# DreamWaterFound/self_commit_ORB-SLAM2

Measured on AMD Instinct MI355X. Metric: frames/s ORB extract+match (1000 feat, 640x480), higher is better.
Workload: dtype u8; 1 GPU; batch of 256 synthetic 640x480 frames per GPU (8 distinct resident batches per step, one launch set per batch), ORB extract (1000 feat, 8 levels, FAST 20/7) + brute-force Hamming SearchByBoW of consecutive frames; batch_per_gpu=256, streams=3, width=640, height=480, nfeatures=1000, parallelism=frames sharded, 1 rank(s), no data-path collective

## Files before the change

### self_commit_orb-slam2_amd/csrc/orbx_match.hip

```cpp
#include <math.h>
#include <string.h>

#include <atomic>
#include <chrono>

#include <type_traits>
#include <vector>

#include "orbx_match_internal.h"

using namespace orbx_match;

namespace {

__global__ __launch_bounds__(256) void k_bow_order(FeatDev A, const int32_t *__restrict__ pairsA, int32_t *__restrict__ order, int stride)
{
    const int p = blockIdx.y, fa = pairsA[p];
    const int nA = min(A.counts[fa], A.cap);
    const int i = blockIdx.x * 256 + threadIdx.x;
    if (i >= nA) return;
    int32_t *ord = order + (size_t)p * stride;
    if (!A.groups) { ord[i] = i; return; }
    const int32_t *g = A.groups + (size_t)fa * A.cap;
    const int gi = g[i];
    int rank = 0;
    for (int k = 0; k < nA; k++) { int gk = g[k]; rank += (gk < gi) || (gk == gi && k < i); }
    ord[rank] = i;
}

#define TOPK_NROW 1
#define TOPK_ROWS (256 * TOPK_NROW)
#define TOPK_TILE 1024

__device__ __forceinline__ uint32_t bcnt_acc(uint32_t x, uint32_t acc)
{
    uint32_t r;
    asm("v_bcnt_u32_b32 %0, %1, %2" : "=v"(r) : "v"(x), "v"(acc));
    return r;
}

struct TriDev {
    const float *f12;
    const float *epipole;
    const uint8_t *stereoA, *stereoB;
    float epiTh[ORBX_MAX_LEVELS];
    double chiTh[ORBX_MAX_LEVELS];
};

__device__ __forceinline__ bool tri_geom_ok(const TriDev &T, int p, const orbx_keypoint &k1, bool st1, const orbx_keypoint &k2, bool st2)
{
    if (!st1 && !st2) {
        const float distex = T.epipole[2 * p] - k2.x, distey = T.epipole[2 * p + 1] - k2.y;
        if (distex * distex + distey * distey < T.epiTh[k2.octave]) return false;
    }
    const float *F = T.f12 + 9 * p;
    const float a = k1.x * F[0] + k1.y * F[3] + F[6];
    const float b = k1.x * F[1] + k1.y * F[4] + F[7];
    const float c = k1.x * F[2] + k1.y * F[5] + F[8];
    const float num = a * k2.x + b * k2.y + c;
    const float den = a * a + b * b;
    if (den == 0) return false;
    const float dsqr = num * num / den;
    return (double)dsqr < T.chiTh[k2.octave];
}

__device__ __forceinline__ uint32_t med3_u32(uint32_t a, uint32_t b, uint32_t c)
{
    uint32_t r;
    asm("v_med3_u32 %0, %1, %2, %3" : "=v"(r) : "v"(a), "v"(b), "v"(c));
    return r;
}

__device__ __forceinline__ void topk_insert(uint32_t (&kk)[TOPK], uint32_t key)
{
#pragma unroll
    for (int q = TOPK - 1; q > 0; q--) kk[q] = med3_u32(kk[q - 1], kk[q], key);
    kk[0] = min(kk[0], key);
}

template <bool FILTER, bool TRI, int NROW>
__global__ __launch_bounds__(256) void k_bow_topk(FeatDev A, FeatDev B, const int32_t *__restrict__ pairsA, const int32_t *__restrict__ pairsB, int mode,
                                                  uint32_t dcut, uint32_t *__restrict__ topk, int stride, TriDev T)
{
    __shared__ uint4 sB[TOPK_TILE * 2];
    __shared__ int32_t sG[TOPK_TILE];
    const int p = blockIdx.y, fa = pairsA[p], fb = pairsB[p];
    const int nA = min(A.counts[fa], A.cap), nB = min(B.counts[fb], B.cap);
    const int capB = B.cap;
    const int row0 = blockIdx.x * (256 * NROW);
    if (row0 >= nA) return;
    const int tid = threadIdx.x;
    int ir[NROW];
    bool live[NROW], act[NROW];
    uint32_t a[NROW][8], kk[NROW][TOPK], th[NROW];
    int gA[NROW];
    const uint32_t sentinel = dcut << 16;
#pragma unroll
    for (int r = 0; r < NROW; r++) {
        ir[r] = row0 + 256 * r + tid;
        live[r] = ir[r] < nA;
        const size_t ia = (size_t)fa * A.cap + (live[r] ? ir[r] : nA - 1);
        const uint32_t *da = (const uint32_t *)(A.desc + ia * 32);
#pragma unroll
        for (int w = 0; w < 8; w++) a[r][w] = da[w];
        gA[r] = (FILTER && A.groups) ? A.groups[ia] : 0;
        act[r] = live[r] && !(FILTER && gA[r] < 0);
#pragma unroll
        for (int q = 0; q < TOPK; q++) kk[r][q] = act[r] ? sentinel : 0u;
        th[r] = kk[r][TOPK - 1] >> 16;
    }
    const uint4 *gD = (const uint4 *)(B.desc + (size_t)fb * capB * 32);
    for (int t0base = 0; t0base < nB; t0base += TOPK_TILE) {
        const int nt = min(TOPK_TILE, nB - t0base), ntPad = (nt + 3) & ~3;
        __syncthreads();
        for (int t = tid; t < 2 * ntPad; t += 256) sB[t] = t < 2 * nt ? gD[2 * (size_t)t0base + t] : make_uint4(0u, 0u, 0u, 0u);
        if (FILTER)
            for (int j = tid; j < ntPad; j += 256) {
                int gq = (int)0x80000000;
                if (j < nt) {
                    gq = B.groups ? B.groups[(size_t)fb * capB + t0base + j] : 0;
                    if (gq < 0) gq = (int)0x80000000;
                    if (mode >= 1 && B.valid && !B.valid[(size_t)fb * capB + t0base + j]) gq = (int)0x80000000;
                }
                sG[j] = gq;
            }
        __syncthreads();
        auto group = [&](const int j0, auto tailTag) {
            constexpr bool TAIL = decltype(tailTag)::value;
            uint32_t dd[NROW][4];
#pragma unroll
            for (int u = 0; u < 4; u++) {
                const uint4 lo = sB[2 * (j0 + u)], hi = sB[2 * (j0 + u) + 1];
                const uint32_t bw[8] = {lo.x, lo.y, lo.z, lo.w, hi.x, hi.y, hi.z, hi.w};
                uint32_t d[NROW];
#pragma unroll
                for (int r = 0; r < NROW; r++) d[r] = bcnt_acc(a[r][0] ^ bw[0], 0u);
#pragma unroll
                for (int w = 1; w < 8; w++)
#pragma unroll
                    for (int r = 0; r < NROW; r++) d[r] = bcnt_acc(a[r][w] ^ bw[w], d[r]);
                if (FILTER) {
                    const int gq = sG[j0 + u];
#pragma unroll
                    for (int r = 0; r < NROW; r++) d[r] = gq == gA[r] ? d[r] : 0xffffu;
                } else if (TAIL && j0 + u >= nt) {
#pragma unroll
                    for (int r = 0; r < NROW; r++) d[r] = 0xffffu;
                }
#pragma unroll
                for (int r = 0; r < NROW; r++) dd[r][u] = d[r];
            }
            auto reaches = [](uint32_t d, uint32_t t) { return TRI ? d <= t : d < t; };
            bool any4 = false;
#pragma unroll
            for (int r = 0; r < NROW; r++) any4 = any4 || reaches(min(min(dd[r][0], min(dd[r][1], dd[r][2])), dd[r][3]), th[r]);
            if (__any(any4)) {
#pragma unroll
                for (int u = 0; u < 4; u++) {
                    bool anyU = false;
#pragma unroll
                    for (int r = 0; r < NROW; r++) anyU = anyU || reaches(dd[r][u], th[r]);
                    if (__any(anyU)) {
                        const uint32_t j = TRI ? 0xffffu - (uint32_t)(t0base + j0 + u) : (uint32_t)(t0base + j0 + u);
                        uint32_t ins[NROW];
#pragma unroll
                        for (int r = 0; r < NROW; r++) ins[r] = (dd[r][u] << 16) | j;
                        if (TRI) {
                            const int jb = t0base + j0 + u;
                            const orbx_keypoint k2 = B.kp[(size_t)fb * capB + jb];
                            const bool st2 = T.stereoB && T.stereoB[(size_t)fb * capB + jb];
#pragma unroll
                            for (int r = 0; r < NROW; r++) {
                                bool pass = false;
                                if (ins[r] < kk[r][TOPK - 1]) {
                                    const size_t ia = (size_t)fa * A.cap + ir[r];
                                    pass = tri_geom_ok(T, p, A.kp[ia], T.stereoA && T.stereoA[ia], k2, st2);
                                }
                                ins[r] = pass ? ins[r] : 0xffffffffu;
                            }
                        }
#pragma unroll
                        for (int r = 0; r < NROW; r++)
                            if (__any(ins[r] < kk[r][TOPK - 1])) { topk_insert(kk[r], ins[r]); th[r] = kk[r][TOPK - 1] >> 16; }
                    }
                }
            }
        };
        int j0 = 0;
        for (; j0 + 4 <= nt; j0 += 4) group(j0, std::false_type());
        if (j0 < ntPad) group(j0, std::true_type());
    }
#pragma unroll
    for (int r = 0; r < NROW; r++)
        if (live[r]) {
            uint32_t *out = topk + ((size_t)p * stride + ir[r]) * TOPK;
#pragma unroll
            for (int k = 0; k < TOPK; k++) out[k] = (!act[r] || kk[r][k] >= sentinel) ? KEY_EMPTY : kk[r][k];
        }
}

typedef int mfma_v4i __attribute__((ext_vector_type(4)));
typedef int mfma_v16i __attribute__((ext_vector_type(16)));

__device__ __forceinline__ uint32_t nib01(uint32_t n) { return __umul24(n, 0x00204081u) & 0x01010101u; }

__global__ __launch_bounds__(256, 3) void k_bow_topk_mfma(FeatDev A, FeatDev B, const int32_t *__restrict__ pairsA, const int32_t *__restrict__ pairsB, uint32_t dcut,
                                                       uint32_t *__restrict__ topk, int stride, int dbg)
{
    __shared__ uint32_t sLut[16 * 64];
    const int p = blockIdx.y, fa = pairsA[p], fb = pairsB[p];
    const int nA = min(A.counts[fa], A.cap), nB = min(B.counts[fb], B.cap);
    const int capB = B.cap;
    const int row0 = blockIdx.x * 256;
    if (row0 >= nA) return;
    const int tid = threadIdx.x, lane = tid & 63, wv = tid >> 6, g = lane >> 5, c = lane & 31;
    for (int e = tid; e < 16 * 64; e += 256) sLut[e] = nib01((uint32_t)e >> 6);
    __syncthreads();
    if (row0 + 64 * wv >= nA) return;
    const uint32_t sentinel = dcut << 16;
    const char *lut = (const char *)sLut;
    const uint32_t lane4 = (uint32_t)lane << 2;
    mfma_v4i a[2][8];
    uint32_t kk[2][TOPK];
    int iA[2], nAc[2], T[2];
    bool live[2];
#pragma unroll
    for (int s = 0; s < 2; s++) {
        iA[s] = row0 + 64 * wv + 32 * s + c;
        live[s] = iA[s] < nA;
        const uint4 *da = (const uint4 *)(A.desc + ((size_t)fa * A.cap + (live[s] ? iA[s] : nA - 1)) * 32);
        const uint4 lo = da[0], hi = da[1];
        nAc[s] = __popc(lo.x) + __popc(lo.y) + __popc(lo.z) + __popc(lo.w) + __popc(hi.x) + __popc(hi.y) + __popc(hi.z) + __popc(hi.w);
        const uint4 mine = g ? hi : lo;
        const uint32_t w[4] = {mine.x, mine.y, mine.z, mine.w};
#pragma unroll
        for (int t = 0; t < 8; t++) {
            const uint32_t two = (w[t >> 1] >> (16 * (t & 1))) & 0xffffu;
#pragma unroll
            for (int q = 0; q < 4; q++) a[s][t][q] = (int)__builtin_amdgcn_perm(0u, 0x0000ff01u, nib01((two >> (4 * q)) & 15u));
        }
#pragma unroll
        for (int q = 0; q < TOPK; q++) kk[s][q] = live[s] ? sentinel : 0u;
        T[s] = (int)(kk[s][TOPK - 1] >> 16) - nAc[s];
    }
    const uint4 *gD = (const uint4 *)(B.desc + (size_t)fb * capB * 32);
    const int ntiles = (nB + 31) >> 5;
    auto load_raw = [&](int tile) { const int j = tile * 32 + c; return j < nB ? gD[(size_t)j * 2 + g] : make_uint4(0u, 0u, 0u, 0u); };
    uint4 raw = load_raw(0);
    auto one_tile = [&](const int tile, auto lastTag) {
        constexpr bool LAST = decltype(lastTag)::value;
// ... 802 lines not shown
    int ndev = 0;
    if (hipGetDeviceCount(&ndev) != hipSuccess || ndev <= 0) { orbx_set_error("no HIP device available: liborbx has no CPU fallback"); return ORBX_ERR_NODEVICE; }
    if (device < 0 || device >= ndev) { orbx_set_error("device %d out of range", device); return ORBX_ERR_ARG; }
    ORBX_HIP_CHECK(hipSetDevice(device));
    orbx_matcher *m = new orbx_matcher();
    m->device = device; m->maxFeatures = max_features; m->maxPairs = max_pairs;
    if (hipStreamCreateWithFlags(&m->stream, hipStreamNonBlocking) != hipSuccess) { delete m; orbx_set_error("hipStreamCreate failed"); return ORBX_ERR_HIP; }
    (void)hipEventCreateWithFlags(&m->evDep, hipEventDisableTiming);
    (void)hipEventCreateWithFlags(&m->evDep2, hipEventDisableTiming);
    (void)hipEventCreateWithFlags(&m->evPyr[0], hipEventDisableTiming);
    (void)hipEventCreateWithFlags(&m->evPyr[1], hipEventDisableTiming);
    (void)hipEventCreateWithFlags(&m->evDone[0], hipEventDisableTiming);
    (void)hipEventCreateWithFlags(&m->evDone[1], hipEventDisableTiming);
    for (int r = 0; r < MATCH_PROF_RING; r++) { (void)hipEventCreate(&m->ev0[r]); (void)hipEventCreate(&m->ev1[r]); (void)hipEventCreate(&m->evMid[r]); }
    const size_t S = (size_t)max_features, P = (size_t)max_pairs;
    int rc;
    if ((rc = m->pairsA.ensure(P)) || (rc = m->pairsB.ensure(P)) || (rc = m->order.ensure(P * S)) || (rc = m->matches.ensure(P * S)) ||
        (rc = m->dists.ensure(P * S)) || (rc = m->nmatches.ensure(P)) || (rc = m->topk.ensure(P * S * TOPK)) || (rc = m->scales.ensure(128)) ||
        (rc = m->uright.ensure(P * S)) || (rc = m->depth.ensure(P * S)) || (rc = m->sad.ensure(P * S))) {
        orbx_matcher_destroy(m);
        return rc;
    }
    *out = m;
    return ORBX_OK;
}

extern "C" void orbx_matcher_destroy(orbx_matcher *m)
{
    if (!m) return;
    (void)hipSetDevice(m->device);
    if (m->stream) (void)hipStreamSynchronize(m->stream);
    m->pairsA.release(); m->pairsB.release(); m->order.release(); m->matches.release(); m->dists.release(); m->nmatches.release();
    m->hostStage.release(); m->projDec.release(); m->projQueue.release(); m->box.release(); m->arena.release();
    m->topk.release(); m->scales.release(); m->uright.release(); m->depth.release(); m->sad.release(); m->stRowStart.release(); m->stRowList.release();
    m->topk64.release(); m->pkp.release(); m->producerStatus.release();
    for (int q = 0; q < 2; q++) { m->pf[q].release(); m->pb[q].release(); m->pi32[q].release(); }
    if (m->evDep2) (void)hipEventDestroy(m->evDep2);
    m->sfZero.release(); m->sfScalesDev.release();
    if (m->sfHost) (void)hipHostFree(m->sfHost);
    for (int i = 0; i < 2; i++) if (m->evPyr[i]) (void)hipEventDestroy(m->evPyr[i]);
    for (int s = 0; s < 2; s++) { m->hk[s].release(); m->hd[s].release(); m->hv[s].release(); m->hc[s].release(); m->hg[s].release(); m->hs[s].release(); }
    m->triGeom.release(); m->frProj.release(); m->frLevel.release(); m->frInView.release();
    if (m->evDep) (void)hipEventDestroy(m->evDep);
    for (int i = 0; i < 2; i++) if (m->evDone[i]) (void)hipEventDestroy(m->evDone[i]);
    for (int r = 0; r < MATCH_PROF_RING; r++) { if (m->ev0[r]) (void)hipEventDestroy(m->ev0[r]); if (m->ev1[r]) (void)hipEventDestroy(m->ev1[r]); if (m->evMid[r]) (void)hipEventDestroy(m->evMid[r]); }
    if (m->stream) (void)hipStreamDestroy(m->stream);
    delete m;
}

__global__ void k_status_or(int *dst, const int *src, int first) { if (first) *dst = *src; else if (*src) atomicOr(dst, *src); }

namespace orbx_match {

int inherit_status(orbx_matcher *m, orbx_extractor *after, bool first)
{
    if (!after) return ORBX_OK;
    const int *w = orbx_extractor_status_word_internal(after);
    if (!w) return ORBX_OK;
    if (!m->producerStatus.p) {
        int rc = m->producerStatus.ensure(1);
        if (rc != ORBX_OK) return rc;
        ORBX_HIP_CHECK(hipMemsetAsync(m->producerStatus.p, 0, sizeof(int), m->stream));
    }
    hipLaunchKernelGGL(k_status_or, dim3(1), dim3(1), 0, m->stream, m->producerStatus.p, w, first ? 1 : 0);
    return ORBX_OK;
}

int check_producer_status(orbx_matcher *m)
{
    if (!m->producerStatus.p) return ORBX_OK;
    int v = 0;
    ORBX_HIP_CHECK(hipMemcpy(&v, m->producerStatus.p, sizeof(int), hipMemcpyDeviceToHost));
    if (!v) return ORBX_OK;
    ORBX_HIP_CHECK(hipMemset(m->producerStatus.p, 0, sizeof(int)));
    orbx_set_error("the extractor batch these results were computed from overflowed a device capacity (bits 0x%x: 1 = >%d FAST candidates in a level, "
                   "2 = quadtree node list, 4 = level keypoints): results are not the reference's", v, 32768);
    return ORBX_ERR_CAPACITY;
}

int prep_pairs(orbx_matcher *m, const orbx_feature_set *a, const orbx_feature_set *b, const int32_t *pa, const int32_t *pb, int npairs,
                      orbx_extractor *after)
{
    if (!m || !a || !b || !pa || !pb) { orbx_set_error("NULL argument"); return ORBX_ERR_ARG; }
    if (npairs < 1 || npairs > m->maxPairs) { orbx_set_error("npairs %d outside 1..%d", npairs, m->maxPairs); return ORBX_ERR_CAPACITY; }
    if (a->capacity > m->maxFeatures || b->capacity > m->maxFeatures || a->capacity < 1 || b->capacity < 1) {
        orbx_set_error("feature capacity %d/%d exceeds the matcher's max_features %d", a->capacity, b->capacity, m->maxFeatures);
        return ORBX_ERR_CAPACITY;
    }
    if (!a->keypoints || !a->descriptors || !a->counts || !b->keypoints || !b->descriptors || !b->counts) { orbx_set_error("NULL feature arrays"); return ORBX_ERR_ARG; }
    for (int p = 0; p < npairs; p++)
        if (pa[p] < 0 || pa[p] >= a->nframes || pb[p] < 0 || pb[p] >= b->nframes) { orbx_set_error("pair %d references a frame out of range", p); return ORBX_ERR_ARG; }
    ORBX_HIP_CHECK(hipSetDevice(m->device));
    if (after) {
        ORBX_HIP_CHECK(hipEventRecord(m->evDep, orbx_extractor_stream_internal(after)));
        ORBX_HIP_CHECK(hipStreamWaitEvent(m->stream, m->evDep, 0));
        int rcs = inherit_status(m, after, true);
        if (rcs != ORBX_OK) return rcs;
    } else if (m->producerStatus.p)
        ORBX_HIP_CHECK(hipMemsetAsync(m->producerStatus.p, 0, sizeof(int), m->stream));
    ORBX_HIP_CHECK(hipMemcpyAsync(m->pairsA.p, pa, (size_t)npairs * sizeof(int32_t), hipMemcpyHostToDevice, m->stream));
    ORBX_HIP_CHECK(hipMemcpyAsync(m->pairsB.p, pb, (size_t)npairs * sizeof(int32_t), hipMemcpyHostToDevice, m->stream));
    return ORBX_OK;
}

int chain_back(orbx_matcher *m, orbx_extractor *after)
{
    if (!after) return ORBX_OK;
    hipEvent_t ev = m->evDone[m->doneSlot];
    m->doneSlot ^= 1;
    ORBX_HIP_CHECK(hipEventRecord(ev, m->stream));
    orbx_extractor_set_consumer_event_internal(after, ev);
    return ORBX_OK;
}

FeatDev to_dev(const orbx_feature_set *s)
{
    FeatDev f;
    f.kp = s->keypoints; f.desc = s->descriptors; f.counts = s->counts; f.groups = s->groups; f.valid = s->valid; f.cap = s->capacity;
    return f;
}

}

extern "C" int orbx_search_by_bow_device(orbx_matcher *m, const orbx_feature_set *a, const orbx_feature_set *b, const int32_t *pairs_a,
                                         const int32_t *pairs_b, int npairs, const orbx_bow_params *params, orbx_extractor *after)
{
    if (!params || (params->mode != 0 && params->mode != 1)) { orbx_set_error("bad bow params"); return ORBX_ERR_ARG; }
    int rc = prep_pairs(m, a, b, pairs_a, pairs_b, npairs, after);
    if (rc != ORBX_OK) return rc;
    const int stride = m->maxFeatures;
    FeatDev A = to_dev(a), B = to_dev(b);
    const int slot = m->profCount % MATCH_PROF_RING;
    ORBX_HIP_CHECK(hipEventRecord(m->ev0[slot], m->stream));
    uint32_t dcut = TH_LOW + 1;
    while (dcut < 257 && !(params->nn_ratio * (float)dcut > (float)TH_LOW)) dcut++;
    const bool filter = b->groups != nullptr || (params->mode == 1 && b->valid != nullptr);
    const dim3 gridTopk((unsigned)((a->capacity + TOPK_ROWS - 1) / TOPK_ROWS), (unsigned)npairs);
    if (filter)
        hipLaunchKernelGGL((k_bow_topk<true, false, TOPK_NROW>), gridTopk, dim3(256), 0, m->stream, A, B, m->pairsA.p, m->pairsB.p, params->mode, dcut, m->topk.p, stride, TriDev());
    else {
        const char *em = getenv("ORBX_MATCH_MFMA");
        const bool mfma = em && em[0] == '1';
        static const int dbg = getenv("ORBX_MFMA_DEBUG") ? atoi(getenv("ORBX_MFMA_DEBUG")) : 0;
        if (mfma) hipLaunchKernelGGL(k_bow_topk_mfma, dim3((unsigned)((a->capacity + 255) / 256), (unsigned)npairs), dim3(256), 0, m->stream, A, B, m->pairsA.p, m->pairsB.p, dcut, m->topk.p, stride, dbg);
        else hipLaunchKernelGGL((k_bow_topk<false, false, TOPK_NROW>), gridTopk, dim3(256), 0, m->stream, A, B, m->pairsA.p, m->pairsB.p, params->mode, dcut, m->topk.p, stride, TriDev());
    }
    MLAUNCH_CHECK();
    ORBX_HIP_CHECK(hipEventRecord(m->evMid[slot], m->stream));
    m->midValid[slot] = true;
    hipLaunchKernelGGL(k_bow_order, dim3((unsigned)((a->capacity + 255) / 256), (unsigned)npairs), dim3(256), 0, m->stream, A, m->pairsA.p, m->order.p, stride);
    MLAUNCH_CHECK();
    const size_t ldsGreedy = (size_t)b->capacity * 4 + (size_t)a->capacity * 4 + (size_t)((a->capacity + 7) & ~7) * 2 * 2;
    if (ldsGreedy > 160 * 1024) { orbx_set_error("feature capacity %d too large for the LDS tile", a->capacity); return ORBX_ERR_CAPACITY; }
    if (ldsGreedy > 48 * 1024) ORBX_HIP_CHECK(hipFuncSetAttribute((const void *)k_bow_greedy, hipFuncAttributeMaxDynamicSharedMemorySize, (int)ldsGreedy));
    hipLaunchKernelGGL(k_bow_greedy, dim3((unsigned)npairs), dim3(GREEDY_THREADS), ldsGreedy, m->stream, A, B, m->pairsA.p, m->pairsB.p, params->mode, params->nn_ratio,
                       params->check_orientation, m->topk.p, m->order.p, m->matches.p, m->dists.p, m->nmatches.p, stride, TriDev(), (int32_t *)nullptr, (unsigned long long *)nullptr, 0ull);
    MLAUNCH_CHECK();
    ORBX_HIP_CHECK(hipEventRecord(m->ev1[slot], m->stream));
    m->profCount++;
    m->lastPairs = npairs; m->lastStride = stride;
    return chain_back(m, after);
}

extern "C" int orbx_stereo_match_device(orbx_matcher *m, const orbx_feature_set *left, const orbx_feature_set *right, const int32_t *pairs_l,
                                        const int32_t *pairs_r, int npairs, const float *scale_factors, int nlevels, float max_disparity,
                                        orbx_extractor *after)
{
    if (!scale_factors || nlevels < 1 || nlevels > 64) { orbx_set_error("bad scale factor table"); return ORBX_ERR_ARG; }
    int rc = prep_pairs(m, left, right, pairs_l, pairs_r, npairs, after);
    if (rc != ORBX_OK) return rc;
    const int stride = m->maxFeatures;
    ORBX_HIP_CHECK(hipMemcpyAsync(m->scales.p, scale_factors, (size_t)nlevels * sizeof(float), hipMemcpyHostToDevice, m->stream));
    ORBX_HIP_CHECK(hipMemsetAsync(m->nmatches.p, 0, (size_t)npairs * sizeof(int32_t), m->stream));
    const int slot = m->profCount % MATCH_PROF_RING;
    ORBX_HIP_CHECK(hipEventRecord(m->ev0[slot], m->stream));
    m->midValid[slot] = false;
    hipLaunchKernelGGL(k_stereo, dim3((unsigned)((left->capacity + 3) / 4), (unsigned)npairs), dim3(256), 0, m->stream, to_dev(left), to_dev(right), m->pairsA.p,
                       m->pairsB.p, m->scales.p, max_disparity, m->matches.p, m->dists.p, m->nmatches.p, stride);
    MLAUNCH_CHECK();
    ORBX_HIP_CHECK(hipEventRecord(m->ev1[slot], m->stream));
    m->profCount++;
    m->lastPairs = npairs; m->lastStride = stride;
    return chain_back(m, after);
}

extern "C" int orbx_compute_stereo_matches_device(orbx_matcher *m, orbx_extractor *left, orbx_extractor *right, const int32_t *frames_l,
                                                  const int32_t *frames_r, int npairs, float mbf, float mb)
{
    if (!m || !left || !right || !frames_l || !frames_r) { orbx_set_error("NULL argument"); return ORBX_ERR_ARG; }
    OrbxLastBatchView vl, vr;
    int rc;
    if ((rc = orbx_extractor_last_batch_view_internal(left, &vl)) != ORBX_OK || (rc = orbx_extractor_last_batch_view_internal(right, &vr)) != ORBX_OK) return rc;
    if (vl.nlevels != vr.nlevels || vl.geom->W != vr.geom->W || vl.geom->H != vr.geom->H) {
        orbx_set_error("left and right extractors differ in geometry (%dx%d/%d vs %dx%d/%d)", vl.geom->W, vl.geom->H, vl.nlevels, vr.geom->W, vr.geom->H, vr.nlevels);
        return ORBX_ERR_ARG;
    }
    if (vl.nlevels > 64) { orbx_set_error("too many levels"); return ORBX_ERR_ARG; }
    orbx_feature_set fl = {vl.kp, vl.desc, vl.counts, nullptr, nullptr, vl.cap, vl.batch};
    orbx_feature_set fr = {vr.kp, vr.desc, vr.counts, nullptr, nullptr, vr.cap, vr.batch};
    rc = prep_pairs(m, &fl, &fr, frames_l, frames_r, npairs, left);
    if (rc != ORBX_OK) return rc;
    if (right != left) {
        ORBX_HIP_CHECK(hipEventRecord(m->evDep2, orbx_extractor_stream_internal(right)));
        ORBX_HIP_CHECK(hipStreamWaitEvent(m->stream, m->evDep2, 0));
// ... 337 lines not shown
    if ((rc = bx.wait(m->stream)) != ORBX_OK) return rc;
    const int32_t *res = bx.outHost<int32_t>(0);
    if (nOut > 0) memcpy(matches, res, (size_t)nOut * 4);
    *nmatches = res[nOut];
    return ORBX_OK;
}

extern "C" int orbx_search_by_bow(orbx_matcher *m, const orbx_feature_set *a_host, const orbx_feature_set *b_host, const orbx_bow_params *params,
                                  int32_t *matches, int32_t *nmatches)
{
    if (!m || !matches || !nmatches) { orbx_set_error("NULL argument"); return ORBX_ERR_ARG; }
    if (!params || (params->mode != 0 && params->mode != 1)) { orbx_set_error("bad bow params"); return ORBX_ERR_ARG; }
    ORBX_HIP_CHECK(hipSetDevice(m->device));
    static const bool split = !(getenv("ORBX_BOW_SINGLE_SPLIT") && getenv("ORBX_BOW_SINGLE_SPLIT")[0] == '0');
    if (split && a_host && b_host && a_host->keypoints && a_host->descriptors && a_host->counts && b_host->keypoints && b_host->descriptors && b_host->counts &&
        a_host->counts[0] > 0 && b_host->counts[0] > 0 && a_host->counts[0] <= m->maxFeatures && b_host->counts[0] <= std::min(m->maxFeatures, 4000))
        return search_by_bow_single(m, a_host, b_host, params, matches, nmatches);
    orbx_feature_set da, db;
    int rc;
    if ((rc = stage_host(m, 0, a_host, &da)) != ORBX_OK || (rc = stage_host(m, 1, b_host, &db)) != ORBX_OK) return rc;
    const int32_t zero = 0;
    if ((rc = orbx_search_by_bow_device(m, &da, &db, &zero, &zero, 1, params, nullptr)) != ORBX_OK) return rc;
    ORBX_HIP_CHECK(hipStreamSynchronize(m->stream));
    const int nOut = params->mode == 0 ? b_host->counts[0] : a_host->counts[0];
    if (nOut > 0) ORBX_HIP_CHECK(hipMemcpy(matches, m->matches.p, (size_t)nOut * 4, hipMemcpyDeviceToHost));
    ORBX_HIP_CHECK(hipMemcpy(nmatches, m->nmatches.p, 4, hipMemcpyDeviceToHost));
    return ORBX_OK;
}

extern "C" int orbx_search_for_triangulation_device(orbx_matcher *m, const orbx_feature_set *a, const orbx_feature_set *b, const int32_t *pairs_a,
                                                    const int32_t *pairs_b, int npairs, const orbx_triangulation_params *params, orbx_extractor *after)
{
    if (!params || !params->f12 || !params->epipole || !params->scale_factors || !params->level_sigma2) { orbx_set_error("bad triangulation params"); return ORBX_ERR_ARG; }
    if (params->nlevels < 1 || params->nlevels > ORBX_MAX_LEVELS) { orbx_set_error("nlevels %d outside 1..%d", params->nlevels, ORBX_MAX_LEVELS); return ORBX_ERR_ARG; }
    int rc = prep_pairs(m, a, b, pairs_a, pairs_b, npairs, after);
    if (rc != ORBX_OK) return rc;
    if ((rc = m->triGeom.ensure((size_t)11 * m->maxPairs)) != ORBX_OK) return rc;
    ORBX_HIP_CHECK(hipMemcpyAsync(m->triGeom.p, params->f12, (size_t)9 * npairs * sizeof(float), hipMemcpyHostToDevice, m->stream));
    ORBX_HIP_CHECK(hipMemcpyAsync(m->triGeom.p + (size_t)9 * m->maxPairs, params->epipole, (size_t)2 * npairs * sizeof(float), hipMemcpyHostToDevice, m->stream));
    TriDev T = TriDev();
    T.f12 = m->triGeom.p; T.epipole = m->triGeom.p + (size_t)9 * m->maxPairs;
    T.stereoA = params->stereo_a; T.stereoB = params->stereo_b;
    for (int l = 0; l < params->nlevels; l++) {
        T.epiTh[l] = 100 * params->scale_factors[l];
        T.chiTh[l] = 3.84 * params->level_sigma2[l];
    }
    const int stride = m->maxFeatures;
    FeatDev A = to_dev(a), B = to_dev(b);
    const int slot = m->profCount % MATCH_PROF_RING;
    ORBX_HIP_CHECK(hipEventRecord(m->ev0[slot], m->stream));
    hipLaunchKernelGGL(k_bow_order, dim3((unsigned)((a->capacity + 255) / 256), (unsigned)npairs), dim3(256), 0, m->stream, A, m->pairsA.p, m->order.p, stride);
    MLAUNCH_CHECK();
    const dim3 gridTopk((unsigned)((a->capacity + TOPK_ROWS - 1) / TOPK_ROWS), (unsigned)npairs);
    hipLaunchKernelGGL((k_bow_topk<true, true, TOPK_NROW>), gridTopk, dim3(256), 0, m->stream, A, B, m->pairsA.p, m->pairsB.p, 2, (uint32_t)(TH_LOW + 1), m->topk.p, stride, T);
    MLAUNCH_CHECK();
    m->midValid[slot] = false;
    const size_t ldsGreedy = (size_t)b->capacity * 4 + (size_t)a->capacity * 4 + (size_t)((a->capacity + 7) & ~7) * 2 * 2;
    if (ldsGreedy > 160 * 1024) { orbx_set_error("feature capacity %d too large for the LDS tile", a->capacity); return ORBX_ERR_CAPACITY; }
    if (ldsGreedy > 48 * 1024) ORBX_HIP_CHECK(hipFuncSetAttribute((const void *)k_bow_greedy, hipFuncAttributeMaxDynamicSharedMemorySize, (int)ldsGreedy));
    hipLaunchKernelGGL(k_bow_greedy, dim3((unsigned)npairs), dim3(GREEDY_THREADS), ldsGreedy, m->stream, A, B, m->pairsA.p, m->pairsB.p, 2, 0.0f, params->check_orientation,
                       m->topk.p, m->order.p, m->matches.p, m->dists.p, m->nmatches.p, stride, T, (int32_t *)nullptr, (unsigned long long *)nullptr, 0ull);
    MLAUNCH_CHECK();
    ORBX_HIP_CHECK(hipEventRecord(m->ev1[slot], m->stream));
    m->profCount++;
    m->lastPairs = npairs; m->lastStride = stride;
    return chain_back(m, after);
}

extern "C" int orbx_search_for_triangulation(orbx_matcher *m, const orbx_feature_set *a_host, const orbx_feature_set *b_host,
                                             const orbx_triangulation_params *params_host, int32_t *matches12, int32_t *nmatches)
{
    if (!m || !params_host || !matches12 || !nmatches) { orbx_set_error("NULL argument"); return ORBX_ERR_ARG; }
    ORBX_HIP_CHECK(hipSetDevice(m->device));
    orbx_feature_set da, db;
    int rc;
    if ((rc = stage_host(m, 0, a_host, &da)) != ORBX_OK || (rc = stage_host(m, 1, b_host, &db)) != ORBX_OK) return rc;
    orbx_triangulation_params P = *params_host;
    const uint8_t *hostFlags[2] = {params_host->stereo_a, params_host->stereo_b};
    const int cnt[2] = {a_host->counts[0], b_host->counts[0]};
    const uint8_t *devFlags[2] = {nullptr, nullptr};
    for (int sd = 0; sd < 2; sd++) {
        if (!hostFlags[sd]) continue;
        if ((rc = m->hs[sd].ensure((size_t)m->maxFeatures)) != ORBX_OK) return rc;
        if (cnt[sd] > 0) ORBX_HIP_CHECK(hipMemcpyAsync(m->hs[sd].p, hostFlags[sd], (size_t)cnt[sd], hipMemcpyHostToDevice, m->stream));
        devFlags[sd] = m->hs[sd].p;
    }
    P.stereo_a = devFlags[0]; P.stereo_b = devFlags[1];
    const int32_t zero = 0;
    if ((rc = orbx_search_for_triangulation_device(m, &da, &db, &zero, &zero, 1, &P, nullptr)) != ORBX_OK) return rc;
    ORBX_HIP_CHECK(hipStreamSynchronize(m->stream));
    if (cnt[0] > 0) ORBX_HIP_CHECK(hipMemcpy(matches12, m->matches.p, (size_t)cnt[0] * 4, hipMemcpyDeviceToHost));
    ORBX_HIP_CHECK(hipMemcpy(nmatches, m->nmatches.p, 4, hipMemcpyDeviceToHost));
    return ORBX_OK;
}

extern "C" int orbx_stereo_match(orbx_matcher *m, const orbx_feature_set *left_host, const orbx_feature_set *right_host, const float *scale_factors,
                                 int nlevels, float max_disparity, int32_t *best_dist, int32_t *best_idx)
{
    if (!m || !best_dist || !best_idx) { orbx_set_error("NULL argument"); return ORBX_ERR_ARG; }
    ORBX_HIP_CHECK(hipSetDevice(m->device));
    orbx_feature_set dl, dr;
    int rc;
    if ((rc = stage_host(m, 0, left_host, &dl)) != ORBX_OK || (rc = stage_host(m, 1, right_host, &dr)) != ORBX_OK) return rc;
    const int32_t zero = 0;
    if ((rc = orbx_stereo_match_device(m, &dl, &dr, &zero, &zero, 1, scale_factors, nlevels, max_disparity, nullptr)) != ORBX_OK) return rc;
    ORBX_HIP_CHECK(hipStreamSynchronize(m->stream));
    const int nL = left_host->counts[0];
// ... 7 lines not shown
```

### self_commit_orb-slam2_amd/csrc/orbx_match_internal.h

```cpp
#ifndef ORBX_MATCH_INTERNAL_H
#define ORBX_MATCH_INTERNAL_H

#include "orbx_internal.h"

#define TH_HIGH 100
#define TH_LOW 50
#define HISTO_LENGTH 30
#define KEY_EMPTY 0xffffffffu
#define TOPK 8
#define MATCH_PROF_RING 64

#define KEY64_EMPTY 0xffffffffffffffffull
#define GRID_COLS 64
#define GRID_ROWS 48

struct FeatDev {
    const orbx_keypoint *kp;
    const uint8_t *desc;
    const int32_t *counts;
    const int32_t *groups;
    const uint8_t *valid;
    int cap;
};

// ... 42 lines not shown
struct orbx_matcher {
    int device = 0, maxFeatures = 0, maxPairs = 0;
    hipStream_t stream = nullptr;
    hipEvent_t evDep = nullptr, evDone[2] = {nullptr, nullptr};
    int doneSlot = 0;
    hipEvent_t ev0[MATCH_PROF_RING] = {}, ev1[MATCH_PROF_RING] = {};
    hipEvent_t evMid[MATCH_PROF_RING] = {};
    bool midValid[MATCH_PROF_RING] = {};
    float lastDistanceMs = 0.f, lastReplayMs = 0.f;
    int profCount = 0;
    OrbxDevBuf<int32_t> pairsA, pairsB, order, matches, dists, nmatches;
    OrbxDevBuf<uint32_t> topk;
    OrbxDevBuf<float> scales, uright, depth, pf[2];
    OrbxDevBuf<unsigned long long> topk64;
    OrbxDevBuf<uint8_t> pb[2];
    OrbxDevBuf<int32_t> pi32[2];
    OrbxDevBuf<orbx_keypoint> pkp;
    OrbxDevBuf<uint32_t> projDec, projQueue;
    OrbxHostStage hostStage;
    OrbxCallBox box;
    OrbxDevBuf<uint8_t> arena;
    OrbxDevBuf<int32_t> sad;
    OrbxDevBuf<int32_t> stRowStart, stRowList;
    hipEvent_t evDep2 = nullptr, evPyr[2] = {nullptr, nullptr};
    int lastStereoPairs = 0;
    float sfScales[128] = {};
    int sfLevels = 0;
    OrbxDevBuf<int32_t> sfZero;
    OrbxDevBuf<float> sfScalesDev;
    float *sfHost = nullptr, *sfHostDev = nullptr;
    size_t sfHostFloats = 0;
    int sfSeq = 0, sfFlagSeq = 0;
    int sfPending = 0;
    OrbxDevBuf<orbx_keypoint> hk[2];
    OrbxDevBuf<uint8_t> hd[2], hv[2];
    OrbxDevBuf<int32_t> hc[2], hg[2];
    OrbxDevBuf<uint8_t> hs[2];
    OrbxDevBuf<float> triGeom;
    OrbxDevBuf<float> frProj;
    OrbxDevBuf<int32_t> frLevel;
    OrbxDevBuf<uint8_t> frInView;
    size_t frCount = 0;
    int lastPairs = 0, lastStride = 0;
    OrbxDevBuf<int> producerStatus;
};

#define MLAUNCH_CHECK()                                                                                              \
    do {                                                                                                             \
        hipError_t e_ = hipGetLastError();                                                                           \
        if (e_ != hipSuccess) { orbx_set_error("kernel launch failed: %s (%s:%d)", hipGetErrorString(e_), __FILE__, __LINE__); return ORBX_ERR_HIP; } \
    } while (0)

namespace orbx_match {
int prep_pairs(orbx_matcher *m, const orbx_feature_set *a, const orbx_feature_set *b, const int32_t *pa, const int32_t *pb, int npairs, orbx_extractor *after);
int chain_back(orbx_matcher *m, orbx_extractor *after);
int inherit_status(orbx_matcher *m, orbx_extractor *after, bool first = true);
int check_producer_status(orbx_matcher *m);
FeatDev to_dev(const orbx_feature_set *s);
int stage_host(orbx_matcher *m, int side, const orbx_feature_set *h, orbx_feature_set *d);
}

#endif
```

Before: 307,500 frames/s.

## Stream B descriptors through scalar loads and fold order/status kernels into top-k

Adds a default unfiltered top-k path that reads frame-B descriptors through wave-uniform scalar (constant address space) loads, double-buffered across groups of four, in place of staging 1024-descriptor tiles in LDS behind barriers. The top-k kernel now also writes the identity order and copies the producer status word, so the separate k_bow_order and k_status_or launches are skipped when there are no groups. This cuts LDS traffic, block barriers and two small launches per batch, but relies on scalar cache bandwidth and manual waitcnt handling. The LDS path remains available through an environment flag.

```diff
diff --git a/self_commit_orb-slam2_amd/csrc/orbx_match.hip b/self_commit_orb-slam2_amd/csrc/orbx_match.hip
--- a/self_commit_orb-slam2_amd/csrc/orbx_match.hip
+++ b/self_commit_orb-slam2_amd/csrc/orbx_match.hip
@@ -29,6 +29,7 @@
 }
 
 #define TOPK_NROW 1
+#define TOPK_SNROW 1
 #define TOPK_ROWS (256 * TOPK_NROW)
 #define TOPK_TILE 1024
 
@@ -78,18 +79,95 @@
     kk[0] = min(kk[0], key);
 }
 
-template <bool FILTER, bool TRI, int NROW>
+typedef uint32_t topk_u32x8 __attribute__((ext_vector_type(8), aligned(4)));
+__device__ __forceinline__ void topk_sload4(uint32_t (&s)[32], const uint8_t *base, int j, int last)
+{
+#pragma unroll
+    for (int u = 0; u < 4; u++) {
+        const int idx = __builtin_amdgcn_readfirstlane(min(j + u, last));
+        const topk_u32x8 v = *(const volatile __attribute__((address_space(4))) topk_u32x8 *)(uintptr_t)(base + (size_t)idx * 32);
+#pragma unroll
+        for (int w = 0; w < 8; w++) s[8 * u + w] = v[w];
+    }
+}
+
+template <bool FILTER, bool TRI, int NROW, bool TAIL, class FetchB, class NodeB>
+__device__ __forceinline__ void topk_group(const uint32_t (&a)[NROW][8], const int (&gA)[NROW], const int (&ir)[NROW], uint32_t (&kk)[NROW][TOPK], uint32_t (&th)[NROW],
+                                           const int jb, const int nLeft, FetchB fetchB, NodeB nodeB, const FeatDev &A, const FeatDev &B, const int fa, const int fb,
+                                           const int p, const TriDev &T)
+{
+    uint32_t dd[NROW][4];
+#pragma unroll
+    for (int u = 0; u < 4; u++) {
+        uint32_t bw[8];
+        fetchB(u, bw);
+        uint32_t d[NROW];
+#pragma unroll
+        for (int r = 0; r < NROW; r++) d[r] = bcnt_acc(a[r][0] ^ bw[0], 0u);
+#pragma unroll
+        for (int w = 1; w < 8; w++)
+#pragma unroll
+            for (int r = 0; r < NROW; r++) d[r] = bcnt_acc(a[r][w] ^ bw[w], d[r]);
+        if (FILTER) {
+            const int gq = nodeB(u);
+#pragma unroll
+            for (int r = 0; r < NROW; r++) d[r] = gq == gA[r] ? d[r] : 0xffffu;
+        } else if (TAIL && u >= nLeft) {
+#pragma unroll
+            for (int r = 0; r < NROW; r++) d[r] = 0xffffu;
+        }
+#pragma unroll
+        for (int r = 0; r < NROW; r++) dd[r][u] = d[r];
+    }
+    auto reaches = [](uint32_t d, uint32_t t) { return TRI ? d <= t : d < t; };
+    bool any4 = false;
+#pragma unroll
+    for (int r = 0; r < NROW; r++) any4 = any4 || reaches(min(min(dd[r][0], min(dd[r][1], dd[r][2])), dd[r][3]), th[r]);
+    if (__any(any4)) {
+#pragma unroll
+        for (int u = 0; u < 4; u++) {
+            bool anyU = false;
+#pragma unroll
+            for (int r = 0; r < NROW; r++) anyU = anyU || reaches(dd[r][u], th[r]);
+            if (__any(anyU)) {
+                const uint32_t j = TRI ? 0xffffu - (uint32_t)(jb + u) : (uint32_t)(jb + u);
+                uint32_t ins[NROW];
+#pragma unroll
+                for (int r = 0; r < NROW; r++) ins[r] = (dd[r][u] << 16) | j;
+                if (TRI) {
+                    const orbx_keypoint k2 = B.kp[(size_t)fb * B.cap + jb + u];
+                    const bool st2 = T.stereoB && T.stereoB[(size_t)fb * B.cap + jb + u];
+#pragma unroll
+                    for (int r = 0; r < NROW; r++) {
+                        bool pass = false;
+                        if (ins[r] < kk[r][TOPK - 1]) {
+                            const size_t ia = (size_t)fa * A.cap + ir[r];
+                            pass = tri_geom_ok(T, p, A.kp[ia], T.stereoA && T.stereoA[ia], k2, st2);
+                        }
+                        ins[r] = pass ? ins[r] : 0xffffffffu;
+                    }
+                }
+#pragma unroll
+                for (int r = 0; r < NROW; r++)
+                    if (__any(ins[r] < kk[r][TOPK - 1])) { topk_insert(kk[r], ins[r]); th[r] = kk[r][TOPK - 1] >> 16; }
+            }
+        }
+    }
+}
+
+template <bool FILTER, bool TRI, int NROW, bool SCALAR>
 __global__ __launch_bounds__(256) void k_bow_topk(FeatDev A, FeatDev B, const int32_t *__restrict__ pairsA, const int32_t *__restrict__ pairsB, int mode,
-                                                  uint32_t dcut, uint32_t *__restrict__ topk, int stride, TriDev T)
-{
-    __shared__ uint4 sB[TOPK_TILE * 2];
-    __shared__ int32_t sG[TOPK_TILE];
+                                                  uint32_t dcut, uint32_t *__restrict__ topk, int stride, TriDev T, int32_t *__restrict__ order,
+                                                  int *__restrict__ statDst, const int *__restrict__ statSrc)
+{
+    static_assert(!SCALAR || (!FILTER && !TRI), "the scalar body is the unfiltered search");
+    const int tid = threadIdx.x;
+    if (statSrc && blockIdx.x == 0 && blockIdx.y == 0 && tid == 0) *statDst = *statSrc;
     const int p = blockIdx.y, fa = pairsA[p], fb = pairsB[p];
     const int nA = min(A.counts[fa], A.cap), nB = min(B.counts[fb], B.cap);
     const int capB = B.cap;
     const int row0 = blockIdx.x * (256 * NROW);
     if (row0 >= nA) return;
-    const int tid = threadIdx.x;
     int ir[NROW];
     bool live[NROW], act[NROW];
     uint32_t a[NROW][8], kk[NROW][TOPK], th[NROW];
@@ -109,86 +187,61 @@
         for (int q = 0; q < TOPK; q++) kk[r][q] = act[r] ? sentinel : 0u;
         th[r] = kk[r][TOPK - 1] >> 16;
     }
-    const uint4 *gD = (const uint4 *)(B.desc + (size_t)fb * capB * 32);
-    for (int t0base = 0; t0base < nB; t0base += TOPK_TILE) {
-        const int nt = min(TOPK_TILE, nB - t0base), ntPad = (nt + 3) & ~3;
-        __syncthreads();
-        for (int t = tid; t < 2 * ntPad; t += 256) sB[t] = t < 2 * nt ? gD[2 * (size_t)t0base + t] : make_uint4(0u, 0u, 0u, 0u);
-        if (FILTER)
-            for (int j = tid; j < ntPad; j += 256) {
-                int gq = (int)0x80000000;
-                if (j < nt) {
-                    gq = B.groups ? B.groups[(size_t)fb * capB + t0base + j] : 0;
-                    if (gq < 0) gq = (int)0x80000000;
-                    if (mode >= 1 && B.valid && !B.valid[(size_t)fb * capB + t0base + j]) gq = (int)0x80000000;
+    if constexpr (SCALAR) {
+        const uint8_t *gB = B.desc + (size_t)fb * capB * 32;
+        const int last = nB - 1;
+        uint32_t s0[32], s1[32];
+        auto none = [](int) { return 0; };
+        auto step = [&](uint32_t (&cur)[32], uint32_t (&nxt)[32], const int j0, auto tailTag) {
+            __builtin_amdgcn_s_waitcnt(0xc07f);
+            topk_sload4(nxt, gB, j0 + 4, last);
+            topk_group<false, false, NROW, decltype(tailTag)::value>(a, gA, ir, kk, th, j0, nB - j0, [&](int u, uint32_t (&bw)[8]) {
+#pragma unroll
+                for (int w = 0; w < 8; w++) bw[w] = cur[8 * u + w];
+            }, none, A, B, fa, fb, p, T);
+        };
+        if (nB > 0) {
+            topk_sload4(s0, gB, 0, last);
+            int j0 = 0;
+            for (; j0 + 8 <= nB; j0 += 8) {
+                step(s0, s1, j0, std::false_type());
+                step(s1, s0, j0 + 4, std::false_type());
+            }
+            if (j0 + 4 <= nB) {
+                step(s0, s1, j0, std::false_type());
+                if (j0 + 4 < nB) step(s1, s0, j0 + 4, std::true_type());
+            } else if (j0 < nB)
+                step(s0, s1, j0, std::true_type());
+        }
+    } else {
+        __shared__ uint4 sB[TOPK_TILE * 2];
+        __shared__ int32_t sG[TOPK_TILE];
+        const uint4 *gD = (const uint4 *)(B.desc + (size_t)fb * capB * 32);
+        for (int t0base = 0; t0base < nB; t0base += TOPK_TILE) {
+            const int nt = min(TOPK_TILE, nB - t0base), ntPad = (nt + 3) & ~3;
+            __syncthreads();
+            for (int t = tid; t < 2 * ntPad; t += 256) sB[t] = t < 2 * nt ? gD[2 * (size_t)t0base + t] : make_uint4(0u, 0u, 0u, 0u);
+            if (FILTER)
+                for (int j = tid; j < ntPad; j += 256) {
+                    int gq = (int)0x80000000;
+                    if (j < nt) {
+                        gq = B.groups ? B.groups[(size_t)fb * capB + t0base + j] : 0;
+                        if (gq < 0) gq = (int)0x80000000;
+                        if (mode >= 1 && B.valid && !B.valid[(size_t)fb * capB + t0base + j]) gq = (int)0x80000000;
+                    }
+                    sG[j] = gq;
                 }
-                sG[j] = gq;
-            }
-        __syncthreads();
-        auto group = [&](const int j0, auto tailTag) {
-            constexpr bool TAIL = decltype(tailTag)::value;
-            uint32_t dd[NROW][4];
-#pragma unroll
-            for (int u = 0; u < 4; u++) {
-                const uint4 lo = sB[2 * (j0 + u)], hi = sB[2 * (j0 + u) + 1];
-                const uint32_t bw[8] = {lo.x, lo.y, lo.z, lo.w, hi.x, hi.y, hi.z, hi.w};
-                uint32_t d[NROW];
-#pragma unroll
-                for (int r = 0; r < NROW; r++) d[r] = bcnt_acc(a[r][0] ^ bw[0], 0u);
-#pragma unroll
-                for (int w = 1; w < 8; w++)
-#pragma unroll
-                    for (int r = 0; r < NROW; r++) d[r] = bcnt_acc(a[r][w] ^ bw[w], d[r]);
-                if (FILTER) {
-                    const int gq = sG[j0 + u];
-#pragma unroll
-                    for (int r = 0; r < NROW; r++) d[r] = gq == gA[r] ? d[r] : 0xffffu;
-                } else if (TAIL && j0 + u >= nt) {
-#pragma unroll
-                    for (int r = 0; r < NROW; r++) d[r] = 0xffffu;
-                }
-#pragma unroll
-                for (int r = 0; r < NROW; r++) dd[r][u] = d[r];
-            }
-            auto reaches = [](uint32_t d, uint32_t t) { return TRI ? d <= t : d < t; };
-            bool any4 = false;
-#pragma unroll
-            for (int r = 0; r < NROW; r++) any4 = any4 || reaches(min(min(dd[r][0], min(dd[r][1], dd[r][2])), dd[r][3]), th[r]);
-            if (__any(any4)) {
-#pragma unroll
-                for (int u = 0; u < 4; u++) {
-                    bool anyU = false;
-#pragma unroll
-                    for (int r = 0; r < NROW; r++) anyU = anyU || reaches(dd[r][u], th[r]);
-                    if (__any(anyU)) {
-                        const uint32_t j = TRI ? 0xffffu - (uint32_t)(t0base + j0 + u) : (uint32_t)(t0base + j0 + u);
-                        uint32_t ins[NROW];
-#pragma unroll
-                        for (int r = 0; r < NROW; r++) ins[r] = (dd[r][u] << 16) | j;
-                        if (TRI) {
-                            const int jb = t0base + j0 + u;
-                            const orbx_keypoint k2 = B.kp[(size_t)fb * capB + jb];
-                            const bool st2 = T.stereoB && T.stereoB[(size_t)fb * capB + jb];
-#pragma unroll
-                            for (int r = 0; r < NROW; r++) {
-                                bool pass = false;
-                                if (ins[r] < kk[r][TOPK - 1]) {
-                                    const size_t ia = (size_t)fa * A.cap + ir[r];
-                                    pass = tri_geom_ok(T, p, A.kp[ia], T.stereoA && T.stereoA[ia], k2, st2);
-                                }
-                                ins[r] = pass ? ins[r] : 0xffffffffu;
-                            }
-                        }
-#pragma unroll
-                        for (int r = 0; r < NROW; r++)
-                            if (__any(ins[r] < kk[r][TOPK - 1])) { topk_insert(kk[r], ins[r]); th[r] = kk[r][TOPK - 1] >> 16; }
-                    }
-                }
-            }
-        };
-        int j0 = 0;
-        for (; j0 + 4 <= nt; j0 += 4) group(j0, std::false_type());
-        if (j0 < ntPad) group(j0, std::true_type());
+            __syncthreads();
+            auto group = [&](const int j0, auto tailTag) {
+                topk_group<FILTER, TRI, NROW, decltype(tailTag)::value>(a, gA, ir, kk, th, t0base + j0, nt - j0, [&](int u, uint32_t (&bw)[8]) {
+                    const uint4 lo = sB[2 * (j0 + u)], hi = sB[2 * (j0 + u) + 1];
+                    bw[0] = lo.x; bw[1] = lo.y; bw[2] = lo.z; bw[3] = lo.w; bw[4] = hi.x; bw[5] = hi.y; bw[6] = hi.z; bw[7] = hi.w;
+                }, [&](int u) { return sG[j0 + u]; }, A, B, fa, fb, p, T);
+            };
+            int j0 = 0;
+            for (; j0 + 4 <= nt; j0 += 4) group(j0, std::false_type());
+            if (j0 < ntPad) group(j0, std::true_type());
+        }
     }
 #pragma unroll
     for (int r = 0; r < NROW; r++)
@@ -196,6 +249,7 @@
             uint32_t *out = topk + ((size_t)p * stride + ir[r]) * TOPK;
 #pragma unroll
             for (int k = 0; k < TOPK; k++) out[k] = (!act[r] || kk[r][k] >= sentinel) ? KEY_EMPTY : kk[r][k];
+            if (order && !A.groups) order[(size_t)p * stride + ir[r]] = ir[r];
         }
 }
 
@@ -1104,7 +1158,7 @@
 
 namespace orbx_match {
 
-int inherit_status(orbx_matcher *m, orbx_extractor *after, bool first)
+int inherit_status(orbx_matcher *m, orbx_extractor *after, bool first, const int **deferred)
 {
     if (!after) return ORBX_OK;
     const int *w = orbx_extractor_status_word_internal(after);
@@ -1114,6 +1168,7 @@
         if (rc != ORBX_OK) return rc;
         ORBX_HIP_CHECK(hipMemsetAsync(m->producerStatus.p, 0, sizeof(int), m->stream));
     }
+    if (deferred && first) { *deferred = w; return ORBX_OK; }
     hipLaunchKernelGGL(k_status_or, dim3(1), dim3(1), 0, m->stream, m->producerStatus.p, w, first ? 1 : 0);
     return ORBX_OK;
 }
@@ -1131,8 +1186,9 @@
 }
 
 int prep_pairs(orbx_matcher *m, const orbx_feature_set *a, const orbx_feature_set *b, const int32_t *pa, const int32_t *pb, int npairs,
-                      orbx_extractor *after)
-{
+                      orbx_extractor *after, const int **deferredStatus)
+{
+    if (deferredStatus) *deferredStatus = nullptr;
     if (!m || !a || !b || !pa || !pb) { orbx_set_error("NULL argument"); return ORBX_ERR_ARG; }
     if (npairs < 1 || npairs > m->maxPairs) { orbx_set_error("npairs %d outside 1..%d", npairs, m->maxPairs); return ORBX_ERR_CAPACITY; }
     if (a->capacity > m->maxFeatures || b->capacity > m->maxFeatures || a->capacity < 1 || b->capacity < 1) {
@@ -1146,7 +1202,7 @@
     if (after) {
         ORBX_HIP_CHECK(hipEventRecord(m->evDep, orbx_extractor_stream_internal(after)));
         ORBX_HIP_CHECK(hipStreamWaitEvent(m->stream, m->evDep, 0));
-        int rcs = inherit_status(m, after, true);
+        int rcs = inherit_status(m, after, true, deferredStatus);
         if (rcs != ORBX_OK) return rcs;
     } else if (m->producerStatus.p)
         ORBX_HIP_CHECK(hipMemsetAsync(m->producerStatus.p, 0, sizeof(int), m->stream));
@@ -1178,7 +1234,11 @@
                                          const int32_t *pairs_b, int npairs, const orbx_bow_params *params, orbx_extractor *after)
 {
     if (!params || (params->mode != 0 && params->mode != 1)) { orbx_set_error("bad bow params"); return ORBX_ERR_ARG; }
-    int rc = prep_pairs(m, a, b, pairs_a, pairs_b, npairs, after);
+    const bool filter = a && b && (b->groups != nullptr || (params->mode == 1 && b->valid != nullptr));
+    const char *em = getenv("ORBX_MATCH_MFMA"), *el = getenv("ORBX_TOPK_LDS");
+    const bool mfma = !filter && em && em[0] == '1', lds = el && el[0] == '1';
+    const int *statSrc = nullptr;
+    int rc = prep_pairs(m, a, b, pairs_a, pairs_b, npairs, after, mfma ? nullptr : &statSrc);
     if (rc != ORBX_OK) return rc;
     const int stride = m->maxFeatures;
     FeatDev A = to_dev(a), B = to_dev(b);
@@ -1186,22 +1246,27 @@
     ORBX_HIP_CHECK(hipEventRecord(m->ev0[slot], m->stream));
     uint32_t dcut = TH_LOW + 1;
     while (dcut < 257 && !(params->nn_ratio * (float)dcut > (float)TH_LOW)) dcut++;
-    const bool filter = b->groups != nullptr || (params->mode == 1 && b->valid != nullptr);
     const dim3 gridTopk((unsigned)((a->capacity + TOPK_ROWS - 1) / TOPK_ROWS), (unsigned)npairs);
+    int *const statDst = m->producerStatus.p;
     if (filter)
-        hipLaunchKernelGGL((k_bow_topk<true, false, TOPK_NROW>), gridTopk, dim3(256), 0, m->stream, A, B, m->pairsA.p, m->pairsB.p, params->mode, dcut, m->topk.p, stride, TriDev());
-    else {
-        const char *em = getenv("ORBX_MATCH_MFMA");
-        const bool mfma = em && em[0] == '1';
+        hipLaunchKernelGGL((k_bow_topk<true, false, TOPK_NROW, false>), gridTopk, dim3(256), 0, m->stream, A, B, m->pairsA.p, m->pairsB.p, params->mode, dcut, m->topk.p, stride, TriDev(),
+                           m->order.p, statDst, statSrc);
+    else if (mfma) {
         static const int dbg = getenv("ORBX_MFMA_DEBUG") ? atoi(getenv("ORBX_MFMA_DEBUG")) : 0;
-        if (mfma) hipLaunchKernelGGL(k_bow_topk_mfma, dim3((unsigned)((a->capacity + 255) / 256), (unsigned)npairs), dim3(256), 0, m->stream, A, B, m->pairsA.p, m->pairsB.p, dcut, m->topk.p, stride, dbg);
-        else hipLaunchKernelGGL((k_bow_topk<false, false, TOPK_NROW>), gridTopk, dim3(256), 0, m->stream, A, B, m->pairsA.p, m->pairsB.p, params->mode, dcut, m->topk.p, stride, TriDev());
-    }
+        hipLaunchKernelGGL(k_bow_topk_mfma, dim3((unsigned)((a->capacity + 255) / 256), (unsigned)npairs), dim3(256), 0, m->stream, A, B, m->pairsA.p, m->pairsB.p, dcut, m->topk.p, stride, dbg);
+    } else if (lds)
+        hipLaunchKernelGGL((k_bow_topk<false, false, TOPK_NROW, false>), gridTopk, dim3(256), 0, m->stream, A, B, m->pairsA.p, m->pairsB.p, params->mode, dcut, m->topk.p, stride, TriDev(),
+                           m->order.p, statDst, statSrc);
+    else
+        hipLaunchKernelGGL((k_bow_topk<false, false, TOPK_SNROW, true>), dim3((unsigned)((a->capacity + 256 * TOPK_SNROW - 1) / (256 * TOPK_SNROW)), (unsigned)npairs), dim3(256), 0, m->stream,
+                           A, B, m->pairsA.p, m->pairsB.p, params->mode, dcut, m->topk.p, stride, TriDev(), m->order.p, statDst, statSrc);
     MLAUNCH_CHECK();
     ORBX_HIP_CHECK(hipEventRecord(m->evMid[slot], m->stream));
     m->midValid[slot] = true;
-    hipLaunchKernelGGL(k_bow_order, dim3((unsigned)((a->capacity + 255) / 256), (unsigned)npairs), dim3(256), 0, m->stream, A, m->pairsA.p, m->order.p, stride);
-    MLAUNCH_CHECK();
+    if (mfma || A.groups) {
+        hipLaunchKernelGGL(k_bow_order, dim3((unsigned)((a->capacity + 255) / 256), (unsigned)npairs), dim3(256), 0, m->stream, A, m->pairsA.p, m->order.p, stride);
+        MLAUNCH_CHECK();
+    }
     const size_t ldsGreedy = (size_t)b->capacity * 4 + (size_t)a->capacity * 4 + (size_t)((a->capacity + 7) & ~7) * 2 * 2;
     if (ldsGreedy > 160 * 1024) { orbx_set_error("feature capacity %d too large for the LDS tile", a->capacity); return ORBX_ERR_CAPACITY; }
     if (ldsGreedy > 48 * 1024) ORBX_HIP_CHECK(hipFuncSetAttribute((const void *)k_bow_greedy, hipFuncAttributeMaxDynamicSharedMemorySize, (int)ldsGreedy));
@@ -1645,7 +1710,8 @@
     hipLaunchKernelGGL(k_bow_order, dim3((unsigned)((a->capacity + 255) / 256), (unsigned)npairs), dim3(256), 0, m->stream, A, m->pairsA.p, m->order.p, stride);
     MLAUNCH_CHECK();
     const dim3 gridTopk((unsigned)((a->capacity + TOPK_ROWS - 1) / TOPK_ROWS), (unsigned)npairs);
-    hipLaunchKernelGGL((k_bow_topk<true, true, TOPK_NROW>), gridTopk, dim3(256), 0, m->stream, A, B, m->pairsA.p, m->pairsB.p, 2, (uint32_t)(TH_LOW + 1), m->topk.p, stride, T);
+    hipLaunchKernelGGL((k_bow_topk<true, true, TOPK_NROW, false>), gridTopk, dim3(256), 0, m->stream, A, B, m->pairsA.p, m->pairsB.p, 2, (uint32_t)(TH_LOW + 1), m->topk.p, stride, T,
+                       (int32_t *)nullptr, (int *)nullptr, (const int *)nullptr);
     MLAUNCH_CHECK();
     m->midValid[slot] = false;
     const size_t ldsGreedy = (size_t)b->capacity * 4 + (size_t)a->capacity * 4 + (size_t)((a->capacity + 7) & ~7) * 2 * 2;
diff --git a/self_commit_orb-slam2_amd/csrc/orbx_match_internal.h b/self_commit_orb-slam2_amd/csrc/orbx_match_internal.h
--- a/self_commit_orb-slam2_amd/csrc/orbx_match_internal.h
+++ b/self_commit_orb-slam2_amd/csrc/orbx_match_internal.h
@@ -118,9 +118,10 @@
     } while (0)
 
 namespace orbx_match {
-int prep_pairs(orbx_matcher *m, const orbx_feature_set *a, const orbx_feature_set *b, const int32_t *pa, const int32_t *pb, int npairs, orbx_extractor *after);
+int prep_pairs(orbx_matcher *m, const orbx_feature_set *a, const orbx_feature_set *b, const int32_t *pa, const int32_t *pb, int npairs, orbx_extractor *after,
+               const int **deferredStatus = nullptr);
 int chain_back(orbx_matcher *m, orbx_extractor *after);
-int inherit_status(orbx_matcher *m, orbx_extractor *after, bool first = true);
+int inherit_status(orbx_matcher *m, orbx_extractor *after, bool first = true, const int **deferred = nullptr);
 int check_producer_status(orbx_matcher *m);
 FeatDev to_dev(const orbx_feature_set *s);
 int stage_host(orbx_matcher *m, int side, const orbx_feature_set *h, orbx_feature_set *d);
```

Result: no change. 308,900 frames/s (median of 4 runs) (+0.5%).
